# silencht/SG-SLAM

Hardware: AMD Instinct MI355X
Metric: tracked frames/sec (640x480 RGB-D) (higher is better)
Workload: dtype u8/f32(bf16x3 matrix products)/f64

## Files before the change

### include/sgx_debug.h

```cpp
#ifndef SGX_DEBUG_H
#define SGX_DEBUG_H
#include "sgx.h"
#ifdef __cplusplus
extern "C" {
#endif

int sgx_orb_debug_level_geometry(const sgx_orb *h, int level, int32_t *w, int32_t *hgt, int32_t *stride);
int sgx_orb_debug_set_unfused_pyramid(int on);
int sgx_orb_debug_read_level(sgx_orb *h, int frame, int level, uint8_t *dst );
int sgx_orb_debug_read_candidates(sgx_orb *h, int frame, int level, int32_t *x, int32_t *y, int32_t *score, int cap, int *n);
int sgx_debug_flow_affine_batch_dev(int batch, int cap, const sgx_keypoint *d_keys, const int32_t *d_n, const float *d_A, const float *d_shift, const float *d_boxes,
                                    int max_boxes, float *d_prev_xy, void *stream);
int sgx_pose_opt_debug_set_threads(int threads_per_frame);
int sgx_ba_debug_last_plan(int32_t plan[4]);
int sgx_ba_debug_set_init(int mode);
int sgx_ba_debug_set_jobs(int host);
int sgx_ba_debug_set_solver(int mode);
int sgx_det_debug_read_blob(sgx_det *h, const char *blob_name, int image, float *dst, int cap, int *n);
int sgx_flow_debug_read_level(sgx_flow *h, int slot, int frame, int level, uint8_t *img);
int sgx_flow_debug_read_slot(sgx_flow *h, int slot, int frame, int level, uint8_t *img, int32_t *pitch);
int sgx_flow_debug_level_size(const sgx_flow *h, int level, int32_t *w, int32_t *hgt);
int sgx_pnp_debug_betas(int which, const double *L, const double *rho, double *betas);
int sgx_debug_corun_bf16(int blocks, int iters, int launches, void *stream);
int sgx_det_debug_detection_output(sgx_det *h, const float *loc, const float *conf, int batch, sgx_det_result *results);
int sgx_det_debug_continued(sgx_det *h, int *count);
int sgx_det_debug_set_fusion(int on);
int sgx_det_debug_set_irb(int on);
int sgx_det_debug_set_block_fusion(int on);
int sgx_det_debug_set_gemm(int mode);
int sgx_det_debug_set_legacy_kernels(int on);
int sgx_det_debug_time_ops(sgx_det *h, const uint8_t *d_img, int pitch, int batch, int reps, float *ms, int cap, int *nops);
// ... 8 lines not shown
```

### sg_slam_amd/capi.py

```python
import ctypes as C
import numpy as np

KP_DTYPE = np.dtype([('x', 'f4'), ('y', 'f4'), ('size', 'f4'), ('angle', 'f4'), ('response', 'f4'),
                     ('octave', 'i4'), ('class_id', 'i4')])


class SgxError(RuntimeError):
    pass


class Camera(C.Structure):
    _fields_ = [('fx', C.c_float), ('fy', C.c_float), ('cx', C.c_float), ('cy', C.c_float), ('bf', C.c_float),
                ('min_x', C.c_float), ('max_x', C.c_float), ('min_y', C.c_float), ('max_y', C.c_float)]


class BaProblem(C.Structure):
    _fields_ = [('n_poses', C.c_int32), ('n_points', C.c_int32), ('n_edges', C.c_int32), ('poses', C.c_void_p), ('pose_fixed', C.c_void_p),
                ('points', C.c_void_p), ('edge_pose', C.c_void_p), ('edge_point', C.c_void_p), ('edge_obs', C.c_void_p), ('edge_info', C.c_void_p)]


class BaStats(C.Structure):
    _fields_ = [('iterations_first', C.c_int32), ('iterations_second', C.c_int32), ('free_poses', C.c_int32), ('reserved', C.c_int32),
                ('chi2_first', C.c_double), ('chi2_second', C.c_double)]

# ... 37 lines not shown
    'sgx_orb_extract_batch_dev', 'sgx_orb_extract', 'sgx_orb_last_status', 'sgx_profile_enable', 'sgx_profile_num_classes', 'sgx_profile_class_name',
    'sgx_profile_read', 'sgx_match_project_frame_batch_dev', 'sgx_match_project_frame', 'sgx_match_project_local_batch_dev',
    'sgx_match_project_local', 'sgx_frame_stereo_from_rgbd_batch_dev', 'sgx_frame_unproject_batch_dev', 'sgx_frame_make_map_points_batch_dev',
    'sgx_frame_merge_matches_batch_dev', 'sgx_pose_optimization_batch_dev', 'sgx_pose_optimization', 'sgx_frame_motion_model_batch_dev',
    'sgx_local_bundle_adjustment', 'sgx_bundle_adjustment', 'sgx_det_create', 'sgx_det_destroy', 'sgx_det_info', 'sgx_det_detect',
    'sgx_det_detect_batch_dev', 'sgx_det_forward_batch_dev', 'sgx_frame_compact_keys_batch_dev', 'sgx_frame_gray_from_color_batch_dev',
    'sgx_det_gemm_mode', 'sgx_det_plan_step', 'sgx_dynamic_mask_batch_dev', 'sgx_tracker_create', 'sgx_tracker_destroy',
    'sgx_tracker_keypoint_capacity', 'sgx_tracker_record_bytes', 'sgx_tracker_set_initial_pose', 'sgx_tracker_step_dev', 'sgx_tracker_host_buffers',
    'sgx_tracker_step_host', 'sgx_tracker_wait_inputs', 'sgx_tracker_sync', 'sgx_tracker_read', 'sgx_tracker_snapshot_pose_dev',
    'sgx_tracker_snapshot_boxes_dev', 'sgx_tracker_pack_records_dev', 'sgx_tracker_frame_dev', 'sgx_tracker_extractor', 'sgx_flow_create',
    'sgx_dist_unique_id', 'sgx_dist_create', 'sgx_dist_destroy', 'sgx_dist_world', 'sgx_dist_gather_records',
    'sgx_flow_destroy', 'sgx_flow_reset', 'sgx_flow_levels', 'sgx_flow_lk_batch_dev', 'sgx_flow_lk', 'sgx_fundamental_ransac_batch_dev',
    'sgx_find_fundamental_mat', 'sgx_hamming_matrix', 'sgx_hamming_matrix_dev', 'sgx_match_search_for_triangulation', 'sgx_match_search_by_bow',
    'sgx_match_search_by_bow_kf', 'sgx_match_fuse_search', 'sgx_match_project_keyframe', 'sgx_match_fuse_search_sim3',
    'sgx_triangulate_new_map_points', 'sgx_mappoint_update_normal_and_depth', 'sgx_mappoint_distinctive_descriptors', 'sgx_sim3_solver_create',
    'sgx_sim3_solver_set_ransac_parameters', 'sgx_sim3_solver_iterate', 'sgx_sim3_solver_get_estimate', 'sgx_sim3_solver_destroy',
    'sgx_match_search_for_initialization', 'sgx_voc_load', 'sgx_voc_create', 'sgx_voc_info', 'sgx_voc_destroy', 'sgx_voc_transform',
    'sgx_voc_transform_batch_dev', 'sgx_voc_score', 'sgx_match_project_sim3', 'sgx_match_search_by_sim3', 'sgx_optimize_sim3',
    'sgx_optimize_essential_graph', 'sgx_correct_map_points', 'sgx_undistort_points', 'sgx_frame_undistort_stereo_rgbd_batch_dev', 'sgx_frame_image_bounds',
    'sgx_tracker_set_distortion', 'sgx_tracker_frame_keys_un_dev', 'sgx_pnp_solver_create', 'sgx_pnp_solver_set_ransac_parameters', 'sgx_pnp_solver_iterate',
    'sgx_pnp_solver_get_estimate', 'sgx_pnp_solver_destroy', 'sgx_pnp_batch_create', 'sgx_pnp_batch_set_dev', 'sgx_pnp_batch_iterate_dev', 'sgx_pnp_batch_destroy',
]
TAP_SYMBOLS = [
    'sgx_orb_debug_level_geometry', 'sgx_orb_debug_set_unfused_pyramid', 'sgx_orb_debug_read_level', 'sgx_orb_debug_read_candidates',
    'sgx_orb_debug_run_octree', 'sgx_pose_opt_debug_set_threads', 'sgx_ba_debug_set_solver', 'sgx_ba_debug_set_jobs', 'sgx_ba_debug_set_init', 'sgx_ba_debug_last_plan', 'sgx_det_debug_read_blob',
    'sgx_det_debug_detection_output', 'sgx_det_debug_continued', 'sgx_debug_flow_affine_batch_dev', 'sgx_det_debug_set_fusion', 'sgx_det_debug_set_legacy_kernels',
    'sgx_det_debug_set_block_fusion', 'sgx_det_debug_set_irb', 'sgx_det_debug_set_gemm', 'sgx_det_debug_time_ops', 'sgx_det_debug_run_step', 'sgx_flow_debug_read_level',
    'sgx_flow_debug_level_size', 'sgx_flow_debug_read_slot', 'sgx_debug_corun_bf16', 'sgx_pnp_debug_betas',
]


def _vp(x):
    if x is None:
        return None
    if isinstance(x, int):
        return C.c_void_p(x)
    if hasattr(x, 'data_ptr'):
        return C.c_void_p(x.data_ptr())
    return x.ctypes.data_as(C.c_void_p)


class SgxLib:
    def __init__(self, path):
        self.path = path
        self.dll = C.CDLL(path)
        d = self.dll
        d.sgx_version.restype = C.c_char_p
# ... 99 lines not shown
        d.sgx_pnp_batch_destroy.argtypes = [vp]; d.sgx_pnp_batch_destroy.restype = None
        d.sgx_mappoint_update_normal_and_depth.argtypes = [C.c_int] + [vp] * 6 + [C.c_int, vp, vp, vp]
        d.sgx_mappoint_distinctive_descriptors.argtypes = [C.c_int, vp, vp, vp, vp]
        d.sgx_triangulate_new_map_points.argtypes = [C.c_int, vp] + [C.c_int] + [vp] * 5 + [C.c_int] + [vp] * 5 + [vp, vp, vp, C.c_int, vp, vp, vp]
        d.sgx_voc_load.argtypes = [C.c_char_p, vp]
        d.sgx_voc_create.argtypes = [C.c_int] * 5 + [vp] * 5
        d.sgx_voc_info.argtypes = [vp] * 7
        d.sgx_voc_destroy.argtypes = [vp]; d.sgx_voc_destroy.restype = None
        d.sgx_voc_transform.argtypes = [vp, C.c_int, vp, C.c_int, vp, vp, vp, vp, vp]
        d.sgx_voc_transform_batch_dev.argtypes = [vp, vp, C.c_size_t, vp, C.c_int, C.c_int, C.c_int, vp, vp, vp, vp]
        d.sgx_voc_score.argtypes = [vp, C.c_int, vp, vp, C.c_int, vp, vp, vp]
        d.sgx_match_search_by_bow_kf.argtypes = [C.c_int] + [vp] * 4 + [C.c_int] + [vp] * 4 + [C.c_float, C.c_int, vp, vp]
        d.sgx_match_fuse_search.argtypes = [C.c_int] + [vp] * 4 + [C.c_int] + [vp] * 6 + [C.POINTER(Camera), vp, vp, C.c_int, C.c_float, C.c_float, vp, vp, vp]
        d.sgx_hamming_matrix_dev.argtypes = [vp, C.c_int, vp, C.c_int, vp, vp]
        d.sgx_match_search_for_triangulation.argtypes = [C.c_int] + [vp] * 6 + [C.c_int] + [vp] * 6 + [vp, C.POINTER(Camera), vp, vp, C.c_int, C.c_int, C.c_int, vp, vp]

        self.has_taps = hasattr(d, 'sgx_det_debug_read_blob')
        if self.has_taps:
            d.sgx_orb_debug_level_geometry.argtypes = [C.c_void_p, C.c_int] + [C.POINTER(C.c_int32)] * 3
            d.sgx_orb_debug_read_level.argtypes = [C.c_void_p, C.c_int, C.c_int, C.c_void_p]
            d.sgx_orb_debug_read_candidates.argtypes = [C.c_void_p, C.c_int, C.c_int, C.c_void_p, C.c_void_p, C.c_void_p, C.c_int, C.POINTER(C.c_int)]
            d.sgx_orb_debug_run_octree.argtypes = [C.c_void_p, C.c_int, C.c_void_p, C.c_int, C.c_void_p, C.c_int, C.POINTER(C.c_int)]
            d.sgx_orb_debug_set_unfused_pyramid.argtypes = [C.c_int]
            d.sgx_pose_opt_debug_set_threads.argtypes = [C.c_int]
            d.sgx_ba_debug_set_solver.argtypes = [C.c_int]
            d.sgx_ba_debug_set_jobs.argtypes = [C.c_int]
            d.sgx_ba_debug_set_init.argtypes = [C.c_int]
            d.sgx_ba_debug_last_plan.argtypes = [C.c_void_p]
            d.sgx_det_debug_detection_output.argtypes = [vp, vp, vp, C.c_int, C.POINTER(DetResult)]
            d.sgx_det_debug_continued.argtypes = [vp, C.POINTER(C.c_int)]
            d.sgx_det_debug_read_blob.argtypes = [vp, C.c_char_p, C.c_int, vp, C.c_int, C.POINTER(C.c_int)]
            for nm in ('fusion', 'legacy_kernels', 'block_fusion', 'irb', 'gemm'):
                getattr(d, 'sgx_det_debug_set_' + nm).argtypes = [C.c_int]
            d.sgx_det_debug_time_ops.argtypes = [vp, vp, C.c_int, C.c_int, C.c_int, vp, C.c_int, C.POINTER(C.c_int)]
            d.sgx_det_debug_run_step.argtypes = [vp, vp, C.c_int, C.c_int, C.c_int, C.c_int, vp]
            d.sgx_debug_flow_affine_batch_dev.argtypes = [C.c_int, C.c_int, vp, vp, vp, vp, vp, C.c_int, vp, vp]
            d.sgx_flow_debug_read_level.argtypes = [vp, C.c_int, C.c_int, C.c_int, vp]
            d.sgx_debug_corun_bf16.argtypes = [C.c_int, C.c_int, C.c_int, vp]
            d.sgx_pnp_debug_betas.argtypes = [C.c_int, vp, vp, vp]
            d.sgx_flow_debug_level_size.argtypes = [vp, C.c_int, C.POINTER(C.c_int32), C.POINTER(C.c_int32)]
            d.sgx_flow_debug_read_slot.argtypes = [vp, C.c_int, C.c_int, C.c_int, vp, C.POINTER(C.c_int32)]

    def tap(self, name):
        if not self.has_taps:
            raise SgxError(f'{name}: {self.path} is the product build and has no test taps; use tests/taps/libsgx_taps.so (make -C sg_slam_amd/csrc taps)')
        return getattr(self.dll, name)
# ... 17 lines not shown
```

### sg_slam_amd/csrc/sgx_flow_kernels.h

```cpp
#pragma once
#include "sgx_rt.h"
#include "sgx_block.h"
#include "sgx_lane.h"
#include <float.h>
#include <math.h>

#define SGX_LK_MAXL 4
#define SGX_LK_WIN 21
#define SGX_LK_TILE_PITCH 36
struct SgxLkGeom {
    int nl;
    int w[SGX_LK_MAXL], h[SGX_LK_MAXL], pitch[SGX_LK_MAXL];
    unsigned ioff[SGX_LK_MAXL];
    unsigned img_stride;
};

SGX_DEV int sgx_reflect101(int p, int len)
{
    if (len == 1) return 0;
    while (p < 0 || p >= len) { if (p < 0) p = -p; else p = 2 * len - 2 - p; }
    return p;
}
SGX_DEV int sgx_floor_f(float v) { return (int)floorf(v); }
SGX_DEV float sgx_i64_to_f32(long long v)
// ... 230 lines not shown
        float ox, oy; uint8_t st;
        sgx_lk_track_point(g, A.cur_img + (size_t)f * g.img_stride, A.prev_img + (size_t)f * g.img_stride, kpt[0], kpt[1], A.max_count, A.eps2, A.min_eig, &ox, &oy, &st);
        A.prev_xy[2 * ((size_t)f * A.cap + kp)] = ox; A.prev_xy[2 * ((size_t)f * A.cap + kp) + 1] = oy;
        if (A.status) A.status[(size_t)f * A.cap + kp] = st;
    }
    SGX_THREADS_END
}
#else
SGX_DEV int sgx_wave_sum_i32(int v)
{
    v += __builtin_amdgcn_update_dpp(0, v, 0xB1, 0xF, 0xF, true);
    v += __builtin_amdgcn_update_dpp(0, v, 0x4E, 0xF, 0xF, true);
    v += __builtin_amdgcn_update_dpp(0, v, 0x124, 0xF, 0xF, true);
    v += __builtin_amdgcn_update_dpp(0, v, 0x128, 0xF, 0xF, true);
    v += __builtin_amdgcn_update_dpp(0, v, 0x142, 0xA, 0xF, false);
    v += __builtin_amdgcn_update_dpp(0, v, 0x143, 0xC, 0xF, false);
    return __builtin_amdgcn_readlane(v, 63);
}
SGX_DEV float sgx_wave_sum_f32(int v)
{
    const int lo = sgx_wave_sum_i32(v & 0xFFFF), hi = sgx_wave_sum_i32(v >> 16);
    return fmaf((float)hi, 65536.0f, (float)lo);
}
SGX_DEV int sgx_mul24(int a, int b) { return __mul24(a, b); }
SGX_DEV int sgx_reflect1(int p, int len) { p = p < 0 ? -p : p; p = p >= len ? 2 * len - 2 - p : p; return min(max(p, 0), len - 1); }

typedef short sgx_i16x2 __attribute__((ext_vector_type(2)));
typedef unsigned short sgx_u16x2 __attribute__((ext_vector_type(2)));
SGX_DEV sgx_i16x2 sgx_as_i16x2(uint32_t v) { return __builtin_bit_cast(sgx_i16x2, v); }
SGX_DEV uint32_t sgx_as_u32(sgx_i16x2 v) { return __builtin_bit_cast(uint32_t, v); }
#define SGX_LK_PAIR(hi, lo, a, b) sgx_as_i16x2(__builtin_amdgcn_perm((hi), (lo), (uint32_t)(a) | 0x0c00u | ((uint32_t)(b) << 16) | 0x0c000000u))
SGX_DEV sgx_i16x2 sgx_lk_next(sgx_i16x2 p, sgx_i16x2 q) { return sgx_as_i16x2(__builtin_amdgcn_alignbit(sgx_as_u32(q), sgx_as_u32(p), 16)); }
#if defined(SGX_LK_NODOT) && !defined(SGX_EMU)
SGX_DEV int sgx_lk_dot2_mad(sgx_i16x2 a, sgx_i16x2 b, int c)
{
    const uint32_t ua = __builtin_bit_cast(uint32_t, a), ub = __builtin_bit_cast(uint32_t, b);
    asm("v_mad_i32_i16 %0, %1, %2, %0 op_sel:[0,0,0,0]" : "+v"(c) : "v"(ua), "v"(ub));
    asm("v_mad_i32_i16 %0, %1, %2, %0 op_sel:[1,1,0,0]" : "+v"(c) : "v"(ua), "v"(ub));
    return c;
}
#define SGX_LK_DOT2(a, b, c) sgx_lk_dot2_mad((a), (b), (c))
#else
#define SGX_LK_DOT2(a, b, c) __builtin_amdgcn_sdot2((a), (b), (c), false)
#endif
SGX_DEV int sgx_lk_dot2_keep(sgx_i16x2 a, sgx_i16x2 b, int c) { return SGX_LK_DOT2(a, b, c); }

template <int PASSES>
// ... 801 lines not shown
```

### sg_slam_amd/csrc/sgx_lane.h

```cpp
#pragma once
#include "sgx_rt.h"

SGX_DEV uint32_t sgx_alignbyte(uint32_t hi, uint32_t lo, int sh)
{
#ifndef SGX_EMU
    return __builtin_amdgcn_alignbyte(hi, lo, (uint32_t)sh);
#else
    return (uint32_t)((((unsigned long long)hi << 32) | lo) >> (8 * sh));
#endif
}

SGX_DEV uint32_t sgx_udot4(uint32_t a, uint32_t b, uint32_t c)
{
#ifndef SGX_EMU
    return __builtin_amdgcn_udot4(a, b, c, false);
#else
    for (int i = 0; i < 4; i++) c += ((a >> (8 * i)) & 255u) * ((b >> (8 * i)) & 255u);
    return c;
#endif
}
SGX_DEV uint32_t sgx_udot2(uint32_t a, uint32_t b, uint32_t c)
{
#ifndef SGX_EMU
    typedef unsigned short sgx_us2 __attribute__((ext_vector_type(2)));
// ... 3 lines not shown
#endif
}

SGX_DEV uint32_t sgx_perm(uint32_t hi, uint32_t lo, uint32_t sel)
{
#ifndef SGX_EMU
    return __builtin_amdgcn_perm(hi, lo, sel);
#else
    const unsigned long long v = ((unsigned long long)hi << 32) | lo;
    uint32_t r = 0;
    for (int i = 0; i < 4; i++) { const uint32_t s = (sel >> (8 * i)) & 255u; if (s < 8u) r |= (uint32_t)((v >> (8 * s)) & 255u) << (8 * i); }
    return r;
#endif
}

SGX_DEV uint32_t sgx_umul24(uint32_t a, uint32_t b)
{
#ifndef SGX_EMU
    return __umul24(a, b);
#else
    return a * b;
#endif
}
```

### sg_slam_amd/csrc/sgx_orb.cpp

```cpp
#include "sgx_orb_kernels.h"
#include "sgx_prof.h"
#include "../../include/sgx.h"
#ifdef SGX_DEBUG_TAPS
#include "../../include/sgx_debug.h"
#endif
#include "../../include/sgx_orb_pattern.h"
#include <math.h>
#include <stdio.h>
#include <stdlib.h>
#include <string.h>
#include <vector>

#ifdef SGX_EMU
thread_local sgx_dim3 blockIdx, blockDim, gridDim;
#endif


struct sgx_orb {
    sgx_orb_config cfg;
    SgxOrbGeom g;
    float scale[SGX_MAX_LEVELS], inv_scale[SGX_MAX_LEVELS], sigma2[SGX_MAX_LEVELS], inv_sigma2[SGX_MAX_LEVELS];
    int umax_h[16];
    SgxCell *d_cells = nullptr;
    SgxXTab *d_xt[SGX_MAX_LEVELS] = {};
    SgxYTab *d_yt[SGX_MAX_LEVELS] = {};
    SgxXGroup *d_xg_all = nullptr; SgxYTab *d_yt_all = nullptr; SgxPyrRect *d_pyr_rects = nullptr; SgxPyrTabs pyr_tabs; int pyr_tiles = 0, pyr_lds = 0;
    int *d_umax = nullptr;
    signed char *d_pattern = nullptr;
    uint8_t *d_pyr = nullptr;
    uint8_t *d_blur = nullptr; SgxBlurTile *d_blur_tiles = nullptr;
    uint32_t *d_cand = nullptr;
    int *d_cand_count = nullptr;
    uint16_t *d_node_scratch = nullptr;
    uint32_t *d_sel = nullptr;
    int *d_sel_count = nullptr;
    uint32_t *d_status = nullptr;
    uint8_t *d_gray1 = nullptr; uint8_t *d_kps1 = nullptr; uint8_t *d_desc1 = nullptr; int *d_count1 = nullptr;
    int last_batch = 0;
    int oct_maxlim = 0;
};

static thread_local int g_orb_unfused_pyramid = 0;
SGX_TAP int sgx_orb_debug_set_unfused_pyramid(int on) { g_orb_unfused_pyramid = on ? 1 : 0; return SGX_OK; }

static inline int cvround_f(float v) { return (int)lrintf(v); }
static inline int cvround_d(double v) { return (int)lrint(v); }

static void build_tables(sgx_orb *h)
{
    const sgx_orb_config &c = h->cfg;
    const double sf = (double)c.scale_factor;
    const int nl = c.nlevels;
    h->scale[0] = 1.0f; h->sigma2[0] = 1.0f;
    for (int i = 1; i < nl; i++) { h->scale[i] = (float)((double)h->scale[i - 1] * sf); h->sigma2[i] = h->scale[i] * h->scale[i]; }
    for (int i = 0; i < nl; i++) { h->inv_scale[i] = 1.0f / h->scale[i]; h->inv_sigma2[i] = 1.0f / h->sigma2[i]; }
    const float factor = (float)(1.0f / sf);
    float want = c.nfeatures * (1 - factor) / (1 - (float)pow((double)factor, (double)nl));
    int sum = 0;
    for (int l = 0; l < nl - 1; l++) { h->g.lv[l].quota = cvround_f(want); sum += h->g.lv[l].quota; want *= factor; }
    h->g.lv[nl - 1].quota = c.nfeatures - sum > 0 ? c.nfeatures - sum : 0;
    int umax[17] = {0};
    const int HP = 15;
    const int vmax = (int)floor(HP * sqrtf(2.f) / 2 + 1), vmin = (int)ceil(HP * sqrtf(2.f) / 2);
    for (int v = 0; v <= vmax; ++v) umax[v] = cvround_d(sqrt((double)HP * HP - v * v));
    for (int v = HP, v0 = 0; v >= vmin; --v) { while (umax[v0] == umax[v0 + 1]) ++v0; umax[v] = v0; ++v0; }
    for (int i = 0; i < 16; i++) h->umax_h[i] = umax[i];
// ... 33 lines not shown
}

extern "C" const char *sgx_status_string(int s)
{
    switch (s) {
    case SGX_OK: return "ok";
    case SGX_ERR_INVALID: return "invalid argument";
    case SGX_ERR_UNSUPPORTED: return "unsupported geometry";
    case SGX_ERR_NOMEM: return "out of memory";
    case SGX_ERR_DEVICE: return "HIP runtime error";
    case SGX_ERR_OVERFLOW: return "device buffer overflow";
    default: return "unknown";
    }
}

extern "C" void sgx_orb_destroy(sgx_orb *h)
{
    if (!h) return;
    (void)hipFree(h->d_cells); (void)hipFree(h->d_umax); (void)hipFree(h->d_pattern); (void)hipFree(h->d_pyr); (void)hipFree(h->d_cand);
    (void)hipFree(h->d_cand_count); (void)hipFree(h->d_node_scratch); (void)hipFree(h->d_sel); (void)hipFree(h->d_sel_count); (void)hipFree(h->d_status);
    (void)hipFree(h->d_gray1); (void)hipFree(h->d_kps1); (void)hipFree(h->d_desc1); (void)hipFree(h->d_count1);
    for (int l = 0; l < SGX_MAX_LEVELS; l++) { (void)hipFree(h->d_xt[l]); (void)hipFree(h->d_yt[l]); }
    (void)hipFree(h->d_xg_all); (void)hipFree(h->d_yt_all); (void)hipFree(h->d_pyr_rects); (void)hipFree(h->d_blur); (void)hipFree(h->d_blur_tiles);
    delete h;
}

extern "C" int sgx_orb_create(const sgx_orb_config *cfg, sgx_orb **out)
{
    if (!cfg || !out) return SGX_ERR_INVALID;
    if (cfg->nlevels < 1 || cfg->nlevels > SGX_MAX_LEVELS || cfg->nfeatures < 1 || cfg->width < 64 || cfg->height < 64 ||
        cfg->width > 4000 || cfg->height > 4000 || cfg->max_batch < 1 || !(cfg->scale_factor > 1.0f)) return SGX_ERR_INVALID;
    sgx_orb *h = new sgx_orb();
    h->cfg = *cfg;
    SgxOrbGeom &g = h->g;
    memset(&g, 0, sizeof g);
    g.nlevels = cfg->nlevels; g.W = cfg->width; g.H = cfg->height; g.ini_th = cfg->ini_th_fast; g.min_th = cfg->min_th_fast;
    build_tables(h);
    std::vector<SgxCell> cells;
    int off = 0, kp_cap = 0, cand_off = 0;
    for (int l = 0; l < g.nlevels; l++) {
        SgxLevel &L = g.lv[l];
        L.w = cvround_f((float)cfg->width * h->inv_scale[l]);
        L.h = cvround_f((float)cfg->height * h->inv_scale[l]);
        L.stride = (L.w + 63) & ~63;
        L.scale = h->scale[l];
        L.patch_size = (int)(31 * h->scale[l]);
// ... 44 lines not shown
        for (const SgxCell &cc : cells) { if (cc.cw > mw) mw = cc.cw; if (cc.ch > mh) mh = cc.ch; }
        const int tile_b = mh * SGX_TILE_STRIDE, q_b = ((mw - 6) * (mh - 6) * 2 + 15) & ~15, o_b = (((mw - 5) / 2) * ((mh - 5) / 2) * 4 + 15) & ~15;
        g.fast_off_score = tile_b; g.fast_off_qlist = 2 * tile_b; g.fast_off_out = 2 * tile_b + q_b; g.fast_lds_bytes = 2 * tile_b + q_b + o_b;
    }
    g.pyr_pitch = (off + 255) & ~255;
    std::vector<SgxBlurTile> btiles;
    {
        int boff = 0;
        for (int l = 0; l < g.nlevels; l++) {
            SgxLevel &L = g.lv[l];
            L.bstride = (L.w + 63) & ~63; L.boff = boff; boff += L.bstride * L.h;
            for (int y0 = 0; y0 < L.h; y0 += SGX_BT_H) for (int x0 = 0; x0 < L.w; x0 += SGX_BT_W) {
                SgxBlurTile t; memset(&t, 0, sizeof t);
                t.level = (short)l; t.x0 = (short)x0; t.y0 = (short)y0; t.w = (short)std::min(SGX_BT_W, L.w - x0); t.h = (short)std::min(SGX_BT_H, L.h - y0);
                btiles.push_back(t);
            }
        }
        g.blur_pitch = (boff + 255) & ~255; g.nblur_tiles = (int)btiles.size();
    }
    g.ncells = (int)cells.size();
    g.kp_cap = kp_cap;

    const int B = cfg->max_batch, nl = g.nlevels;
#define SGX_ALLOC(p, bytes) do { if (hipMalloc((void **)&(p), (bytes)) != hipSuccess) { sgx_orb_destroy(h); return SGX_ERR_NOMEM; } } while (0)
    SGX_ALLOC(h->d_cells, cells.size() * sizeof(SgxCell));
    SGX_ALLOC(h->d_umax, 16 * sizeof(int));
    SGX_ALLOC(h->d_pattern, 1024);
    SGX_ALLOC(h->d_pyr, (size_t)B * g.pyr_pitch + 256);
    SGX_ALLOC(h->d_blur, (size_t)B * g.blur_pitch + 256);
    SGX_ALLOC(h->d_blur_tiles, btiles.size() * sizeof(SgxBlurTile));
    SGX_CHECK_HIP(hipMemcpy(h->d_blur_tiles, btiles.data(), btiles.size() * sizeof(SgxBlurTile), hipMemcpyHostToDevice));
    SGX_ALLOC(h->d_cand, (size_t)B * g.cand_pitch * 4);
    SGX_ALLOC(h->d_node_scratch, (size_t)B * g.cand_pitch * 2);
    SGX_ALLOC(h->d_cand_count, (size_t)B * nl * 4);
    SGX_ALLOC(h->d_sel, (size_t)B * nl * SGX_OCT_MAXN * 4);
    SGX_ALLOC(h->d_sel_count, (size_t)B * nl * 4);
    SGX_ALLOC(h->d_status, 4);
    SGX_ALLOC(h->d_gray1, (size_t)((g.W + 3) & ~3) * g.H);
    SGX_ALLOC(h->d_kps1, (size_t)kp_cap * 28);
    SGX_ALLOC(h->d_desc1, (size_t)kp_cap * 32);
    SGX_ALLOC(h->d_count1, 4);
    SGX_CHECK_HIP(hipMemcpyAsync(h->d_cells, cells.data(), cells.size() * sizeof(SgxCell), hipMemcpyHostToDevice, 0));
    SGX_CHECK_HIP(hipMemcpyAsync(h->d_umax, h->umax_h, 16 * sizeof(int), hipMemcpyHostToDevice, 0));
    SGX_CHECK_HIP(hipMemcpyAsync(h->d_pattern, sgx_orb_pattern_xy, 1024, hipMemcpyHostToDevice, 0));
    SGX_CHECK_HIP(hipMemsetAsync(h->d_status, 0, 4, 0));
    for (int l = 1; l < nl; l++) {
        std::vector<SgxXTab> xt; std::vector<SgxYTab> yt;
        build_resize_tables(g.lv[l - 1].w, g.lv[l - 1].h, g.lv[l].w, g.lv[l].h, xt, yt);
        SGX_ALLOC(h->d_xt[l], xt.size() * sizeof(SgxXTab));
        SGX_ALLOC(h->d_yt[l], yt.size() * sizeof(SgxYTab));
        SGX_CHECK_HIP(hipMemcpyAsync(h->d_xt[l], xt.data(), xt.size() * sizeof(SgxXTab), hipMemcpyHostToDevice, 0));
        SGX_CHECK_HIP(hipMemcpyAsync(h->d_yt[l], yt.data(), yt.size() * sizeof(SgxYTab), hipMemcpyHostToDevice, 0));
        SGX_CHECK_HIP(hipStreamSynchronize(0));
    }
    SGX_CHECK_HIP(hipStreamSynchronize(0));
    if (nl > 1) {
        std::vector<std::vector<SgxXTab>> xts(nl); std::vector<std::vector<SgxYTab>> yts(nl);
        std::vector<SgxXGroup> xall; std::vector<SgxYTab> yall;
        bool span_ok = true;
        memset(&h->pyr_tabs, 0, sizeof h->pyr_tabs);
        for (int l = 1; l < nl; l++) {
            build_resize_tables(g.lv[l - 1].w, g.lv[l - 1].h, g.lv[l].w, g.lv[l].h, xts[l], yts[l]);
            h->pyr_tabs.xoff[l] = (int)xall.size(); h->pyr_tabs.yoff[l] = (int)yall.size();
            yall.insert(yall.end(), yts[l].begin(), yts[l].end());
            for (int x4 = 0; x4 < g.lv[l].w; x4 += 4) {
                SgxXGroup G; memset(&G, 0, sizeof G);
                G.sx0 = xts[l][x4].sx;
                for (int i = 0; i < 4; i++) {
// ... 96 lines not shown
    const int nl = g.nlevels;
    h->last_batch = batch;
    SGX_CHECK_HIP(hipMemsetAsync(h->d_cand_count, 0, (size_t)batch * nl * 4, stream));
    sgx_prof_begin(SGX_K_RESIZE, stream);
    static const int pyr_threads = sgx_getenv("SGX_TUNE_PYR_THREADS") ? atoi(sgx_getenv("SGX_TUNE_PYR_THREADS")) : 512;
    if (h->pyr_tiles > 0 && !g_orb_unfused_pyramid)
        SGX_LAUNCH_DYN(k_pyramid, dim3(h->pyr_tiles, batch), dim3(pyr_threads), h->pyr_lds, stream, g, h->pyr_tabs, d_gray, pitch, h->d_pyr, h->d_xg_all, h->d_yt_all, h->d_pyr_rects);
    else
        for (int l = 1; l < nl; l++) {
            dim3 grid((g.lv[l].w + 255) / 256, (g.lv[l].h + 3) / 4, batch);
            SGX_LAUNCH(k_resize, grid, dim3(256), stream, g, l, d_gray, pitch, h->d_pyr, h->d_xt[l], h->d_yt[l]);
        }
    sgx_prof_end(SGX_K_RESIZE, stream);
    sgx_prof_begin(SGX_K_FAST, stream);
    static const int fast_threads = sgx_getenv("SGX_TUNE_FAST_THREADS") ? atoi(sgx_getenv("SGX_TUNE_FAST_THREADS")) : 128;
    static const int e_extra = sgx_getenv("SGX_TUNE_E_EXTRA_LDS") ? atoi(sgx_getenv("SGX_TUNE_E_EXTRA_LDS")) : 0;
    SGX_LAUNCH_DYN(k_fast_cells, dim3(g.ncells * batch), dim3(fast_threads), g.fast_lds_bytes + e_extra, stream, g, h->d_cells, d_gray, pitch, h->d_pyr, batch,
               h->d_cand, h->d_cand_count, h->d_status);
    sgx_prof_end(SGX_K_FAST, stream);
    sgx_prof_begin(SGX_K_OCTREE, stream);
    launch_octree(h, batch, stream);
    sgx_prof_end(SGX_K_OCTREE, stream);
    sgx_prof_begin(SGX_K_ORIENT_DESC, stream);
    unsigned long long umax_packed = 0;
    for (int i = 0; i < 16; i++) umax_packed |= (unsigned long long)(h->umax_h[i] & 15) << (4 * i);
#ifdef SGX_DEBUG_TAPS
    static const bool patch_blur = sgx_getenv("SGX_TUNE_ORB_PATCH_BLUR") != nullptr;
    if (patch_blur) {
        SGX_LAUNCH_DYN(k_orient_desc, dim3(g.kp_cap * batch), dim3(64), e_extra / 2, stream, g, d_gray, pitch, h->d_pyr, h->d_sel, h->d_sel_count,
                       umax_packed, h->d_pattern, (uint8_t *)d_kps, d_desc, d_count, cap, batch, h->d_status);
    } else
#endif
    {
        static const int blur_threads = sgx_getenv("SGX_TUNE_BLUR_THREADS") ? atoi(sgx_getenv("SGX_TUNE_BLUR_THREADS")) : 256;
        {
            const int blur_grid = sgx_getenv("SGX_TUNE_ORB_BLUR_GRID") ? atoi(sgx_getenv("SGX_TUNE_ORB_BLUR_GRID")) : 4096;
            const int parts = std::min(g.nblur_tiles, std::max(1, blur_grid / batch));
            SGX_LAUNCH(k_blur_levels, dim3(parts * batch), dim3(std::min(512, std::max(256, blur_threads))), stream, g, h->d_blur_tiles, d_gray, pitch, h->d_pyr, h->d_blur, batch);
        }
#ifdef SGX_DEBUG_TAPS
        static const bool one_per_wave = sgx_getenv("SGX_TUNE_ORB_DESC_ONE_PER_WAVE") != nullptr;
        if (one_per_wave)
            SGX_LAUNCH(k_orient_desc2, dim3(g.kp_cap * batch), dim3(64), stream, g, d_gray, pitch, h->d_pyr, h->d_blur, h->d_sel, h->d_sel_count,
                       umax_packed, h->d_pattern, (uint8_t *)d_kps, d_desc, d_count, cap, batch, h->d_status);
        else
#endif
            SGX_LAUNCH(k_orient_desc4, dim3(((g.kp_cap + 3) / 4) * batch), dim3(64), stream, g, d_gray, pitch, h->d_pyr, h->d_blur, h->d_sel, h->d_sel_count,
                       umax_packed, h->d_pattern, (uint8_t *)d_kps, d_desc, d_count, cap, batch, h->d_status);
    }
    sgx_prof_end(SGX_K_ORIENT_DESC, stream);
    SGX_CHECK_HIP(hipGetLastError());
    return SGX_OK;
}

extern "C" int sgx_orb_last_status(sgx_orb *h, void *stream_)
{
    if (!h) return SGX_ERR_INVALID;
    uint32_t st = 0;
    SGX_CHECK_HIP(hipMemcpyAsync(&st, h->d_status, 4, hipMemcpyDeviceToHost, (sgx_stream_t)stream_));
    SGX_CHECK_HIP(hipStreamSynchronize((sgx_stream_t)stream_));
    if (st) { SGX_CHECK_HIP(hipMemsetAsync(h->d_status, 0, 4, (sgx_stream_t)stream_)); return SGX_ERR_OVERFLOW; }
    return SGX_OK;
}

extern "C" int sgx_orb_extract(sgx_orb *h, const uint8_t *gray, int stride, sgx_keypoint *kps, uint8_t *desc, int cap, int *n)
{
    if (!h || !gray || !kps || !desc || !n || stride < h->g.W || cap < 0) return SGX_ERR_INVALID;
    const int W = h->g.W, H = h->g.H, kc = h->g.kp_cap, P = (W + 3) & ~3;
    if (stride == P) SGX_CHECK_HIP(hipMemcpyAsync(h->d_gray1, gray, (size_t)P * (H - 1) + W, hipMemcpyHostToDevice, 0));
    else for (int y = 0; y < H; y++)
        SGX_CHECK_HIP(hipMemcpyAsync(h->d_gray1 + (size_t)y * P, gray + (size_t)y * stride, W, hipMemcpyHostToDevice, 0));
// ... 65 lines not shown
```

### sg_slam_amd/csrc/sgx_orb_kernels.h

```cpp
#pragma once
#include "sgx_rt.h"
#include "sgx_block.h"
#include "sgx_lane.h"

#define SGX_MAX_LEVELS 12
#define SGX_EDGE 19
#define SGX_BORDER 16
#define SGX_TILE_MAX 68
#define SGX_TILE_STRIDE 72
#define SGX_CAND_LDS 8192
#define SGX_OCT_MAXN 1280
#define SGX_OCT_THREADS 512

struct SgxLevel {
    int w, h, stride;
    int off;
    int quota;
    int ncols, nrows, wcell, hcell;
    int cell0;
    int patch_size;
    int cand_off, cand_cap;
    int boff, bstride;
    float scale;
};
// ... 1014 lines not shown
    const uint8_t *bl = blur + (size_t)frame * g.blur_pitch + L.boff + (size_t)ky * L.bstride + kx;
#pragma unroll
    for (int it_ = 0; it_ < 4; it_++) { const int t = tid + 64 * it_;
        const uint32_t pw = *(const uint32_t *)(pattern + 4 * t);
        const float x0 = (float)(signed char)(pw & 255u), y0 = (float)(signed char)((pw >> 8) & 255u), x1 = (float)(signed char)((pw >> 16) & 255u), y1 = (float)(signed char)(pw >> 24);
        const int r0 = sgx_cvround(x0 * b + y0 * a), c0 = sgx_cvround(x0 * a - y0 * b);
        const int r1 = sgx_cvround(x1 * b + y1 * a), c1 = sgx_cvround(x1 * a - y1 * b);
        const int t0 = bl[r0 * L.bstride + c0], t1 = bl[r1 * L.bstride + c1];
        bits[t] = (uint8_t)(t0 < t1);
    }
    SGX_THREADS_END
    SGX_SYNC();
    SGX_THREADS_BEGIN(tid)
    if (tid < 32) {
        int v = 0;
#pragma unroll
        for (int j = 0; j < 8; j++) v |= bits[8 * tid + j] << j;
        desc[((size_t)frame * cap + slot) * 32 + tid] = (uint8_t)v;
    }
    SGX_THREADS_END
}
#endif

SGX_KERNEL(64) k_orient_desc4(SgxOrbGeom g, const uint8_t *gray, int gray_pitch, const uint8_t *pyr, const uint8_t *blur,
                              const uint32_t *sel, const int *sel_count, unsigned long long umax_packed, const signed char *pattern,
                              uint8_t *kps_raw, uint8_t *desc, int *count, int cap, int batch, uint32_t *status)
{
    SGX_LDS uint32_t patch_dw[4][31 * SGX_MS / 4];
    SGX_LDS uint8_t bits[4][256];
    SGX_LDS int s_m01[4], s_m10[4];
    SGX_LDS float s_a[4], s_b[4];
    int slot4, frame;
    {
        const int n = (int)blockIdx.x, kc = (g.kp_cap + 3) >> 2;
        if ((batch & 7) == 0) { const int xcd = n & 7, j = n >> 3; frame = xcd + 8 * (j / kc); slot4 = j % kc; }
        else { frame = n / kc; slot4 = n % kc; }
    }
    int total = 0;
    for (int l = 0; l < g.nlevels; l++) total += sel_count[frame * g.nlevels + l];
    if (slot4 == 0) {
        SGX_THREADS_BEGIN(tid)
        if (tid == 0) { count[frame] = total < cap ? total : cap; if (total > cap) sgx_atomic_or(status, SGX_ST_KP_OVERFLOW); }
        SGX_THREADS_END
    }
    if (4 * slot4 >= total || 4 * slot4 >= cap) return;

// ... 93 lines not shown
            const float x0 = (float)(signed char)(pw & 255u), y0 = (float)(signed char)((pw >> 8) & 255u), x1 = (float)(signed char)((pw >> 16) & 255u), y1 = (float)(signed char)(pw >> 24);
            const int r0 = sgx_cvround(x0 * b + y0 * a), c0 = sgx_cvround(x0 * a - y0 * b);
            const int r1 = sgx_cvround(x1 * b + y1 * a), c1 = sgx_cvround(x1 * a - y1 * b);
            const int t0 = bl[r0 * L.bstride + c0], t1 = bl[r1 * L.bstride + c1];
            bits[grp][t] = (uint8_t)(t0 < t1);
        }
    }
    SGX_THREADS_END
    SGX_SYNC();
    SGX_THREADS_BEGIN(tid)
    const int grp = tid >> 4, l16 = tid & 15, slot = 4 * slot4 + grp;
    if (slot < total && slot < cap) {
#pragma unroll
        for (int h2 = 0; h2 < 2; h2++) {
            const int byte = 2 * l16 + h2;
            int v = 0;
#pragma unroll
            for (int j = 0; j < 8; j++) v |= bits[grp][8 * byte + j] << j;
            desc[((size_t)frame * cap + slot) * 32 + byte] = (uint8_t)v;
        }
    }
    SGX_THREADS_END
}
```

Baseline: 29970.

## Replace ORB orient/descriptor kernel with 16-keypoint-per-block dot4 moment kernel

The default orientation and descriptor kernel changes from k_orient_desc4 (4 keypoints per 64-thread block, patch staged in LDS) to k_orient_desc16<4> (16 keypoints per 256-thread block). Moments are computed directly from global rows using precomputed circular-mask words and packed udot4 products. BRIEF bits are built per lane from a lane-sliced float pattern table, with each lane writing two descriptor bytes, so the LDS bit buffer and its packing pass go away. The aim is to cut LDS staging and synchronisation and to amortise per-block setup. The trade-offs are unstaged global loads, which may be unaligned, and a new 32-bit offset limit that is checked at create time.

```diff
diff --git a/include/sgx_debug.h b/include/sgx_debug.h
--- a/include/sgx_debug.h
+++ b/include/sgx_debug.h
@@ -7,6 +7,7 @@
 
 int sgx_orb_debug_level_geometry(const sgx_orb *h, int level, int32_t *w, int32_t *hgt, int32_t *stride);
 int sgx_orb_debug_set_unfused_pyramid(int on);
+int sgx_orb_debug_set_desc_kernel(int which);
 int sgx_orb_debug_read_level(sgx_orb *h, int frame, int level, uint8_t *dst );
 int sgx_orb_debug_read_candidates(sgx_orb *h, int frame, int level, int32_t *x, int32_t *y, int32_t *score, int cap, int *n);
 int sgx_debug_flow_affine_batch_dev(int batch, int cap, const sgx_keypoint *d_keys, const int32_t *d_n, const float *d_A, const float *d_shift, const float *d_boxes,
diff --git a/sg_slam_amd/capi.py b/sg_slam_amd/capi.py
--- a/sg_slam_amd/capi.py
+++ b/sg_slam_amd/capi.py
@@ -83,7 +83,7 @@
     'sgx_pnp_solver_get_estimate', 'sgx_pnp_solver_destroy', 'sgx_pnp_batch_create', 'sgx_pnp_batch_set_dev', 'sgx_pnp_batch_iterate_dev', 'sgx_pnp_batch_destroy',
 ]
 TAP_SYMBOLS = [
-    'sgx_orb_debug_level_geometry', 'sgx_orb_debug_set_unfused_pyramid', 'sgx_orb_debug_read_level', 'sgx_orb_debug_read_candidates',
+    'sgx_orb_debug_level_geometry', 'sgx_orb_debug_set_unfused_pyramid', 'sgx_orb_debug_set_desc_kernel', 'sgx_orb_debug_read_level', 'sgx_orb_debug_read_candidates',
     'sgx_orb_debug_run_octree', 'sgx_pose_opt_debug_set_threads', 'sgx_ba_debug_set_solver', 'sgx_ba_debug_set_jobs', 'sgx_ba_debug_set_init', 'sgx_ba_debug_last_plan', 'sgx_det_debug_read_blob',
     'sgx_det_debug_detection_output', 'sgx_det_debug_continued', 'sgx_debug_flow_affine_batch_dev', 'sgx_det_debug_set_fusion', 'sgx_det_debug_set_legacy_kernels',
     'sgx_det_debug_set_block_fusion', 'sgx_det_debug_set_irb', 'sgx_det_debug_set_gemm', 'sgx_det_debug_time_ops', 'sgx_det_debug_run_step', 'sgx_flow_debug_read_level',
@@ -229,6 +229,7 @@
             d.sgx_orb_debug_read_candidates.argtypes = [C.c_void_p, C.c_int, C.c_int, C.c_void_p, C.c_void_p, C.c_void_p, C.c_int, C.POINTER(C.c_int)]
             d.sgx_orb_debug_run_octree.argtypes = [C.c_void_p, C.c_int, C.c_void_p, C.c_int, C.c_void_p, C.c_int, C.POINTER(C.c_int)]
             d.sgx_orb_debug_set_unfused_pyramid.argtypes = [C.c_int]
+            d.sgx_orb_debug_set_desc_kernel.argtypes = [C.c_int]
             d.sgx_pose_opt_debug_set_threads.argtypes = [C.c_int]
             d.sgx_ba_debug_set_solver.argtypes = [C.c_int]
             d.sgx_ba_debug_set_jobs.argtypes = [C.c_int]
diff --git a/sg_slam_amd/csrc/sgx_flow_kernels.h b/sg_slam_amd/csrc/sgx_flow_kernels.h
--- a/sg_slam_amd/csrc/sgx_flow_kernels.h
+++ b/sg_slam_amd/csrc/sgx_flow_kernels.h
@@ -276,7 +276,6 @@
     const int lo = sgx_wave_sum_i32(v & 0xFFFF), hi = sgx_wave_sum_i32(v >> 16);
     return fmaf((float)hi, 65536.0f, (float)lo);
 }
-SGX_DEV int sgx_mul24(int a, int b) { return __mul24(a, b); }
 SGX_DEV int sgx_reflect1(int p, int len) { p = p < 0 ? -p : p; p = p >= len ? 2 * len - 2 - p : p; return min(max(p, 0), len - 1); }
 
 typedef short sgx_i16x2 __attribute__((ext_vector_type(2)));
diff --git a/sg_slam_amd/csrc/sgx_lane.h b/sg_slam_amd/csrc/sgx_lane.h
--- a/sg_slam_amd/csrc/sgx_lane.h
+++ b/sg_slam_amd/csrc/sgx_lane.h
@@ -49,3 +49,12 @@
     return a * b;
 #endif
 }
+
+SGX_DEV int sgx_mul24(int a, int b)
+{
+#ifndef SGX_EMU
+    return __mul24(a, b);
+#else
+    return a * b;
+#endif
+}
diff --git a/sg_slam_amd/csrc/sgx_orb.cpp b/sg_slam_amd/csrc/sgx_orb.cpp
--- a/sg_slam_amd/csrc/sgx_orb.cpp
+++ b/sg_slam_amd/csrc/sgx_orb.cpp
@@ -27,6 +27,7 @@
     SgxXGroup *d_xg_all = nullptr; SgxYTab *d_yt_all = nullptr; SgxPyrRect *d_pyr_rects = nullptr; SgxPyrTabs pyr_tabs; int pyr_tiles = 0, pyr_lds = 0;
     int *d_umax = nullptr;
     signed char *d_pattern = nullptr;
+    uint32_t *d_mom_mask = nullptr; float *d_pattern_sl = nullptr;
     uint8_t *d_pyr = nullptr;
     uint8_t *d_blur = nullptr; SgxBlurTile *d_blur_tiles = nullptr;
     uint32_t *d_cand = nullptr;
@@ -42,6 +43,8 @@
 
 static thread_local int g_orb_unfused_pyramid = 0;
 SGX_TAP int sgx_orb_debug_set_unfused_pyramid(int on) { g_orb_unfused_pyramid = on ? 1 : 0; return SGX_OK; }
+static thread_local int g_orb_desc_kernel = 0;
+SGX_TAP int sgx_orb_debug_set_desc_kernel(int which) { if (which < 0 || which > 2) return SGX_ERR_INVALID; g_orb_desc_kernel = which; return SGX_OK; }
 
 static inline int cvround_f(float v) { return (int)lrintf(v); }
 static inline int cvround_d(double v) { return (int)lrint(v); }
@@ -121,6 +124,7 @@
     (void)hipFree(h->d_gray1); (void)hipFree(h->d_kps1); (void)hipFree(h->d_desc1); (void)hipFree(h->d_count1);
     for (int l = 0; l < SGX_MAX_LEVELS; l++) { (void)hipFree(h->d_xt[l]); (void)hipFree(h->d_yt[l]); }
     (void)hipFree(h->d_xg_all); (void)hipFree(h->d_yt_all); (void)hipFree(h->d_pyr_rects); (void)hipFree(h->d_blur); (void)hipFree(h->d_blur_tiles);
+    (void)hipFree(h->d_mom_mask); (void)hipFree(h->d_pattern_sl);
     delete h;
 }
 
@@ -211,6 +215,7 @@
     g.kp_cap = kp_cap;
 
     const int B = cfg->max_batch, nl = g.nlevels;
+    if ((size_t)B * g.blur_pitch + 256 > 0xFFFFFFFFull) { sgx_orb_destroy(h); return SGX_ERR_UNSUPPORTED; }
 #define SGX_ALLOC(p, bytes) do { if (hipMalloc((void **)&(p), (bytes)) != hipSuccess) { sgx_orb_destroy(h); return SGX_ERR_NOMEM; } } while (0)
     SGX_ALLOC(h->d_cells, cells.size() * sizeof(SgxCell));
     SGX_ALLOC(h->d_umax, 16 * sizeof(int));
@@ -233,6 +238,18 @@
     SGX_CHECK_HIP(hipMemcpyAsync(h->d_umax, h->umax_h, 16 * sizeof(int), hipMemcpyHostToDevice, 0));
     SGX_CHECK_HIP(hipMemcpyAsync(h->d_pattern, sgx_orb_pattern_xy, 1024, hipMemcpyHostToDevice, 0));
     SGX_CHECK_HIP(hipMemsetAsync(h->d_status, 0, 4, 0));
+    {
+        std::vector<uint32_t> mm(4 * 32 * SGX_MM_ROW, 0u); std::vector<float> ps(1024);
+        for (int lead = 0; lead < 4; lead++) for (int r = 0; r < 31; r++) for (int q = 0; q < 9; q++) for (int j = 0; j < 4; j++) {
+            const int u = 4 * q + j - lead - 15, v = r - 15;
+            if (abs(u) <= h->umax_h[abs(v)]) mm[(lead * 32 + r) * SGX_MM_ROW + q] |= 255u << (8 * j);
+        }
+        for (int st = 0; st < 16; st++) for (int lane = 0; lane < 16; lane++) for (int c = 0; c < 4; c++)
+            ps[4 * (16 * st + lane) + c] = (float)((const signed char *)sgx_orb_pattern_xy)[4 * (16 * lane + st) + c];
+        SGX_ALLOC(h->d_mom_mask, mm.size() * 4); SGX_ALLOC(h->d_pattern_sl, ps.size() * 4);
+        SGX_CHECK_HIP(hipMemcpy(h->d_mom_mask, mm.data(), mm.size() * 4, hipMemcpyHostToDevice));
+        SGX_CHECK_HIP(hipMemcpy(h->d_pattern_sl, ps.data(), ps.size() * 4, hipMemcpyHostToDevice));
+    }
     for (int l = 1; l < nl; l++) {
         std::vector<SgxXTab> xt; std::vector<SgxYTab> yt;
         build_resize_tables(g.lv[l - 1].w, g.lv[l - 1].h, g.lv[l].w, g.lv[l].h, xt, yt);
@@ -375,9 +392,9 @@
     launch_octree(h, batch, stream);
     sgx_prof_end(SGX_K_OCTREE, stream);
     sgx_prof_begin(SGX_K_ORIENT_DESC, stream);
+#ifdef SGX_DEBUG_TAPS
     unsigned long long umax_packed = 0;
     for (int i = 0; i < 16; i++) umax_packed |= (unsigned long long)(h->umax_h[i] & 15) << (4 * i);
-#ifdef SGX_DEBUG_TAPS
     static const bool patch_blur = sgx_getenv("SGX_TUNE_ORB_PATCH_BLUR") != nullptr;
     if (patch_blur) {
         SGX_LAUNCH_DYN(k_orient_desc, dim3(g.kp_cap * batch), dim3(64), e_extra / 2, stream, g, d_gray, pitch, h->d_pyr, h->d_sel, h->d_sel_count,
@@ -396,10 +413,16 @@
         if (one_per_wave)
             SGX_LAUNCH(k_orient_desc2, dim3(g.kp_cap * batch), dim3(64), stream, g, d_gray, pitch, h->d_pyr, h->d_blur, h->d_sel, h->d_sel_count,
                        umax_packed, h->d_pattern, (uint8_t *)d_kps, d_desc, d_count, cap, batch, h->d_status);
+        else if (g_orb_desc_kernel == 1)
+            SGX_LAUNCH(k_orient_desc4, dim3(((g.kp_cap + 3) / 4) * batch), dim3(64), stream, g, d_gray, pitch, h->d_pyr, h->d_blur, h->d_sel, h->d_sel_count,
+                       umax_packed, h->d_pattern, (uint8_t *)d_kps, d_desc, d_count, cap, batch, h->d_status);
+        else if (g_orb_desc_kernel == 2)
+            SGX_LAUNCH(k_orient_desc16<1>, dim3(((g.kp_cap + 15) / 16) * batch), dim3(64), stream, g, d_gray, pitch, h->d_pyr, h->d_blur, h->d_sel, h->d_sel_count,
+                       h->d_mom_mask, h->d_pattern_sl, (uint8_t *)d_kps, d_desc, d_count, cap, batch, h->d_status);
         else
 #endif
-            SGX_LAUNCH(k_orient_desc4, dim3(((g.kp_cap + 3) / 4) * batch), dim3(64), stream, g, d_gray, pitch, h->d_pyr, h->d_blur, h->d_sel, h->d_sel_count,
-                       umax_packed, h->d_pattern, (uint8_t *)d_kps, d_desc, d_count, cap, batch, h->d_status);
+            SGX_LAUNCH(k_orient_desc16<4>, dim3(((g.kp_cap + 15) / 16) * batch), dim3(256), stream, g, d_gray, pitch, h->d_pyr, h->d_blur, h->d_sel, h->d_sel_count,
+                       h->d_mom_mask, h->d_pattern_sl, (uint8_t *)d_kps, d_desc, d_count, cap, batch, h->d_status);
     }
     sgx_prof_end(SGX_K_ORIENT_DESC, stream);
     SGX_CHECK_HIP(hipGetLastError());
diff --git a/sg_slam_amd/csrc/sgx_orb_kernels.h b/sg_slam_amd/csrc/sgx_orb_kernels.h
--- a/sg_slam_amd/csrc/sgx_orb_kernels.h
+++ b/sg_slam_amd/csrc/sgx_orb_kernels.h
@@ -1060,6 +1060,7 @@
 }
 #endif
 
+#ifdef SGX_DEBUG_TAPS
 SGX_KERNEL(64) k_orient_desc4(SgxOrbGeom g, const uint8_t *gray, int gray_pitch, const uint8_t *pyr, const uint8_t *blur,
                               const uint32_t *sel, const int *sel_count, unsigned long long umax_packed, const signed char *pattern,
                               uint8_t *kps_raw, uint8_t *desc, int *count, int cap, int batch, uint32_t *status)
@@ -1199,3 +1200,129 @@
     }
     SGX_THREADS_END
 }
+#endif
+
+#define SGX_MM_ROW 12
+template <int WAVES>
+SGX_KERNEL(64 * WAVES) k_orient_desc16(SgxOrbGeom g, const uint8_t *gray, int gray_pitch, const uint8_t *pyr, const uint8_t *blur,
+                                       const uint32_t *sel, const int *sel_count, const uint32_t *mom_mask, const float *pattern_sl,
+                                       uint8_t *kps_raw, uint8_t *desc, int *count, int cap, int batch, uint32_t *status)
+{
+    SGX_LDS int s_level[16], s_kxy[16], s_rstride[16], s_bstride[16], s_psize[16], s_m01[16], s_m10[16];
+    SGX_LDS uint32_t s_e[16], s_roff[16], s_boff[16];
+    SGX_LDS float s_scale[16], s_a[16], s_b[16];
+    int slot16, frame;
+    {
+        const int n = (int)blockIdx.x, kc = (g.kp_cap + 15) >> 4;
+        if ((batch & 7) == 0) { const int xcd = n & 7, j = n >> 3; frame = xcd + 8 * (j / kc); slot16 = j % kc; }
+        else { frame = n / kc; slot16 = n % kc; }
+    }
+    int total = 0;
+    for (int l = 0; l < g.nlevels; l++) total += sel_count[frame * g.nlevels + l];
+    if (slot16 == 0) {
+        SGX_THREADS_BEGIN(tid)
+        if (tid == 0) { count[frame] = total < cap ? total : cap; if (total > cap) sgx_atomic_or(status, SGX_ST_KP_OVERFLOW); }
+        SGX_THREADS_END
+    }
+    if (16 * slot16 >= total || 16 * slot16 >= cap) return;
+
+    SGX_THREADS_BEGIN(tid)
+    if (tid < 16) {
+        const int slot = 16 * slot16 + tid;
+        int level = -1, base = 0, acc_ = 0, rstride = 0, bstride = 0, psize = 0; uint32_t roff = 0, boff = 0; float scale = 1.f;
+        for (int l = 0; l < g.nlevels; l++) {
+            const int n = sel_count[frame * g.nlevels + l];
+            if (level < 0 && slot < acc_ + n) {
+                level = l; base = acc_;
+                rstride = l == 0 ? gray_pitch : g.lv[l].stride; roff = l == 0 ? 0u : (uint32_t)g.lv[l].off;
+                bstride = g.lv[l].bstride; boff = (uint32_t)g.lv[l].boff; psize = g.lv[l].patch_size; scale = g.lv[l].scale;
+            }
+            acc_ += n;
+        }
+        if (slot >= cap) level = -1;
+        s_level[tid] = level; s_m01[tid] = 0; s_m10[tid] = 0;
+        if (level >= 0) {
+            const uint32_t e = sel[((size_t)frame * g.nlevels + level) * SGX_OCT_MAXN + (slot - base)];
+            const int kx = (int)(e & 0xFFF) + SGX_BORDER, ky = (int)((e >> 12) & 0xFFF) + SGX_BORDER;
+            const int px0 = kx - 15, xa = px0 - (px0 & 3);
+            s_e[tid] = e; s_kxy[tid] = kx | (ky << 16); s_rstride[tid] = rstride; s_bstride[tid] = bstride; s_psize[tid] = psize; s_scale[tid] = scale;
+            s_roff[tid] = roff + (uint32_t)((ky - 15) * rstride + xa);
+            s_boff[tid] = (uint32_t)frame * (uint32_t)g.blur_pitch + boff + (uint32_t)(ky * bstride + kx);
+        }
+    }
+    SGX_THREADS_END
+    SGX_SYNC();
+    SGX_THREADS_BEGIN(tid)
+    const int l16 = tid & 15;
+    const uint8_t *raw0 = gray + (size_t)frame * gray_pitch * g.H, *rawN = pyr + (size_t)frame * g.pyr_pitch;
+    for (int rd = 0; rd < 4 / WAVES; rd++) {
+        const int k = (tid >> 4) + 4 * WAVES * rd, level = s_level[k];
+        if (level >= 0) {
+            const int lead = ((s_kxy[k] & 0xFFFF) - 15) & 3, rstride = s_rstride[k];
+            const uint8_t *p = (level == 0 ? raw0 : rawN) + s_roff[k];
+            uint32_t wa[9];
+            wa[0] = 0x03020100u << (8 * lead); wa[1] = 0x07060504u - 0x01010101u * (uint32_t)lead;
+#pragma unroll
+            for (int q = 2; q < 9; q++) wa[q] = wa[q - 1] + 0x04040404u;
+            uint32_t su = 0, si = 0; int m01 = 0;
+#pragma unroll
+            for (int h2 = 0; h2 < 2; h2++) {
+                const int r = l16 + 16 * h2;
+                if (r < 31) {
+                    const uint32_t *row = (const uint32_t *)(p + (uint32_t)(r * rstride));
+                    const uint32_t *mk = mom_mask + (lead * 32 + r) * SGX_MM_ROW;
+                    uint32_t rowsum = 0;
+#pragma unroll
+                    for (int q = 0; q < 9; q++) {
+                        const uint32_t w = row[q] & mk[q];
+                        su = sgx_udot4(w, wa[q], su); rowsum = sgx_udot4(w, 0x01010101u, rowsum);
+                    }
+                    si += rowsum; m01 += sgx_mul24(r - 15, (int)rowsum);
+                }
+            }
+            sgx_atomic_add(&s_m10[k], (int)su - 15 * (int)si); sgx_atomic_add(&s_m01[k], m01);
+        }
+    }
+    SGX_THREADS_END
+    SGX_SYNC();
+    SGX_THREADS_BEGIN(tid)
+    if (tid < 16 && s_level[tid] >= 0) {
+        const int level = s_level[tid], slot = 16 * slot16 + tid, kx = s_kxy[tid] & 0xFFFF, ky = s_kxy[tid] >> 16;
+        const uint32_t e = s_e[tid];
+        const float angle = sgx_fast_atan2((float)s_m01[tid], (float)s_m10[tid]);
+        const float factorPI = (float)(3.1415926535897932384626433832795 / 180.f);
+        float sn, cs;
+        sgx_sincosf(angle * factorPI, &sn, &cs);
+        s_a[tid] = cs; s_b[tid] = sn;
+        float *kp = (float *)(kps_raw + ((size_t)frame * cap + slot) * 28);
+        float fx = (float)kx, fy = (float)ky;
+        if (level != 0) { fx = fx * s_scale[tid]; fy = fy * s_scale[tid]; }
+        kp[0] = fx; kp[1] = fy; kp[2] = (float)s_psize[tid]; kp[3] = angle; kp[4] = (float)(e >> 24);
+        ((int *)kp)[5] = level; ((int *)kp)[6] = -1;
+    }
+    SGX_THREADS_END
+    SGX_SYNC();
+    SGX_THREADS_BEGIN(tid)
+    const int l16 = tid & 15;
+    for (int rd = 0; rd < 4 / WAVES; rd++) {
+        const int k = (tid >> 4) + 4 * WAVES * rd;
+        if (s_level[k] >= 0) {
+            const int slot = 16 * slot16 + k, bstride = s_bstride[k];
+            const float a = s_a[k], b = s_b[k];
+            const uint32_t bo = s_boff[k];
+            uint32_t v = 0;
+#pragma clang loop vectorize(disable) unroll(full)
+            for (int st = 0; st < 16; st++) {
+                const float *pt = pattern_sl + 4 * (16 * st + l16);
+                const float x0 = pt[0], y0 = pt[1], x1 = pt[2], y1 = pt[3];
+                const int r0 = sgx_cvround(x0 * b + y0 * a), c0 = sgx_cvround(x0 * a - y0 * b);
+                const int r1 = sgx_cvround(x1 * b + y1 * a), c1 = sgx_cvround(x1 * a - y1 * b);
+                const int t0 = blur[bo + (uint32_t)(sgx_mul24(r0, bstride) + c0)], t1 = blur[bo + (uint32_t)(sgx_mul24(r1, bstride) + c1)];
+                v |= (uint32_t)(t0 < t1) << st;
+            }
+            uint8_t *d = desc + ((size_t)frame * cap + slot) * 32 + 2 * l16;
+            d[0] = (uint8_t)v; d[1] = (uint8_t)(v >> 8);
+        }
+    }
+    SGX_THREADS_END
+}
```

Result: no change. 30110 (median of 6 runs) (+0.5%).
